# phaistos-networks/Trinity

Measured on AMD Instinct MI355X. Metric: queries/sec, higher is better.
Workload: dtype u32

## Files before the change

### trinity_amd/csrc/host/plan_host.cpp

```cpp
#include "../planner.hpp"
#include "../lucene_enc_units.hpp"
#include "lucene_encoder.hpp"
#include "perc_lower.hpp"

#include <cstdlib>
#include <memory>
#include <mutex>

namespace {
        struct HostPlan {
                BatchPlan P;
                uint8_t *block = nullptr;
                ~HostPlan() { free(block); }
        };
        void put_err(char *err, size_t cap, const std::string &s) {
                if (err && cap) {
                        const size_t n = std::min(cap - 1, s.size());
                        memcpy(err, s.data(), n);
                        err[n] = 0;
                }
        }
}

extern "C" {
void *tri_host_index_build(const uint8_t *index, uint64_t len, const uint8_t *hits, uint64_t hits_len, int codec, const uint32_t *terms3, uint64_t nterms,
                           uint32_t docs_cnt, char *err, uint64_t errcap) {
        auto H = std::make_unique<HostIndex>();
        std::string e;
        static_assert(sizeof(tri_term) == 12, "tri_term is three u32");
        if (build_host_index(index, len, hits, hits_len, codec, reinterpret_cast<const tri_term *>(terms3), nterms, docs_cnt, *H, e) != TRI_OK) {
                put_err(err, errcap, e);
                return nullptr;
        }
        return H.release();
}
void tri_host_index_free(void *h) { delete static_cast<HostIndex *>(h); }

void *tri_host_plan(void *hindex, const uint32_t *prog, uint64_t prog_len, const uint32_t *queries2, uint64_t nq, uint32_t flags, uint32_t topk, int similarity,
                    unsigned threads, const char *const *opt_names, const uint64_t *opt_values, unsigned nopt, uint32_t cus, char *err, uint64_t errcap) {
        const HostIndex &H = *static_cast<HostIndex *>(hindex);
        PlanEnv env;
        env.cus = cus ? cus : 256;
        bool use_frag_cache = false;
        for (unsigned i = 0; i < nopt; ++i) {
                const std::string n = opt_names[i];
                if (n == "frag_cache") {
                        use_frag_cache = opt_values[i] != 0;
                        continue;
                }
                tri_options &o = env.opt;
                uint64_t *slot = n == "dense_min_postings" ? &o.dense_min_postings : n == "dense_task_cost" ? &o.dense_task_cost : n == "fused" ? &o.fused
                                 : n == "fused_task_cost" ? &o.fused_task_cost : n == "fused_freq_cap" ? &o.fused_freq_cap : n == "fused_halfwords" ? &o.fused_halfwords
                                 : n == "account_needed_bytes" ? &o.account_needed_bytes : n == "planes" ? &o.planes : n == "planes_split" ? &o.planes_split
                                 : n == "plane_div" ? &o.plane_div : n == "plane_max_bytes" ? &o.plane_max_bytes : n == "probe_max_blocks" ? &o.probe_max_blocks : n == "tree_max_bytes" ? &o.tree_max_bytes : n == "tree_max_nodes" ? &o.tree_max_nodes : n == "tree_wide_min_nodes" ? &o.tree_wide_min_nodes : n == "result_bitmaps" ? &o.result_bitmaps : n == "cand_task_cost" ? &o.cand_task_cost : n == "dense_window_cost" ? &o.dense_window_cost
                                 : n == "cand_xcd" ? &o.cand_xcd : n == "planes_order" ? &o.planes_order : n == "pset_order" ? &o.pset_order : n == "scatter_bitmap_slack" ? &o.scatter_bitmap_slack : n == "phrase_task_div" ? &o.phrase_task_div : n == "plane_amortize" ? &o.plane_amortize : n == "rich_max_terms" ? &o.rich_max_terms
                                 : n == "overlap" ? &o.overlap : n == "overlap_dense_wgs" ? &o.overlap_dense_wgs : n == "overlap_cand_wgs" ? &o.overlap_cand_wgs  : nullptr;
                if (!slot) {
                        put_err(err, errcap, "unknown option " + n);
                        return nullptr;
                }
                *slot = opt_values[i];
        }
        PlanInput in;
        in.prog = prog;
        in.prog_len = prog_len;
        static_assert(sizeof(tri_query) == 8, "tri_query is two u32");
        in.queries = reinterpret_cast<const tri_query *>(queries2);
        in.nq = nq;
        in.flags = flags;
        in.topk = topk;
        in.similarity = similarity;
        auto hp = std::make_unique<HostPlan>();
        std::unique_ptr<HostPool> pool;
        if (threads > 1)
                pool = std::make_unique<HostPool>(threads);
        std::string e;
        static trip::FragCache g_frag_cache;
        static std::mutex g_frag_mu;
        std::unique_lock<std::mutex> frag_lock(g_frag_mu, std::defer_lock);
        if (use_frag_cache)
                frag_lock.lock();
        const int rc = plan_batch(
                H, env, in, pool.get(),
                [&](size_t bytes) {
                        hp->block = static_cast<uint8_t *>(aligned_alloc(64, (bytes + 63) & ~(size_t)63));
                        if (hp->block)
                                memset(hp->block, 0, bytes);
                        return hp->block;
                },
                hp->P, e, use_frag_cache ? &g_frag_cache : nullptr);
        if (rc != TRI_OK) {
                put_err(err, errcap, e);
                return nullptr;
        }
        return hp.release();
}
void tri_host_plan_free(void *p) { delete static_cast<HostPlan *>(p); }

void tri_host_plan_summary(void *p, uint64_t *out , double *ms ) {
        const BatchPlan &P = static_cast<HostPlan *>(p)->P;
        const uint64_t v[] = {P.block_bytes,       P.plan.size(),    P.qterms.size(),      P.tasks.size(),  P.fused.size(),       P.qplane.size(),    P.plane_terms.size(), P.sterms.size(),
                              P.sweights.size(),   P.phrases.size(), P.pterms.size(),      P.ptasks.size(), P.plan.off,           P.qterms.off,       P.tasks.off,          P.sched.off,
                              P.fused.off,         P.qplane.off,     P.plane_terms.off,    P.sterms.off,    P.sweights.off,       P.phrases.off,      P.pterms.off,         P.ptasks.off,
                              P.n_dense,           P.n_cand,         P.n_fused,            P.n_fused16,     P.n_fusedgen,         P.n_planes,         P.n_planes8,          P.plw,
                              P.sparse_cap,        P.out_capacity,   P.term_bytes,         P.term_bytes_dense, P.dense_queries,   P.cand_queries,     P.fused_queries,      P.planes_queries,
                              P.unsupported_queries, P.rich_R,       sizeof(DevQuery),     sizeof(DevTask), sizeof(DevFused),     sizeof(DevPhrase),  P.cand_needed_term_bytes, P.plane_decoded_bytes,
                              P.n_pset,            P.pset_queries,   P.n_probe,            P.probe_queries, P.units.size(),       P.units.off,        P.pset_sched.off,     sizeof(DevPsetUnit),
                              P.n_tree,            P.tree_queries,   P.tree.size(),        P.tree.off,      P.tree_terms.size(),  P.tree_terms.off,   P.tree_hidden.size(), P.tree_hidden.off,
// ... 190 lines not shown
```

### trinity_amd/csrc/planner.hpp

```cpp
#pragma once
#include "planner_lower.hpp"
#include "planner_tasks.hpp"

namespace trip {
        struct RowQ {
                uint8_t n = 0, q[CAND_QUEUES] = {}, sub[CAND_QUEUES] = {};
        };
        struct LapTimer {
                const bool on;
                std::chrono::steady_clock::time_point t0 = std::chrono::steady_clock::now();
                std::string line;
                void lap(const char *what) {
                        if (!on)
                                return;
                        char buf[64];
                        snprintf(buf, sizeof buf, " %s %.3f", what, ms_since(t0));
                        line += buf;
                }
        };

        struct PlanState {
                const HostIndex &ix;
                const PlanEnv &env;
                const tri_options &opt;
// ... 235 lines not shown
                        q.out_off += f.b_off;
                        if (f.tmp[i].fuse)
                                q.fused_idx += (uint32_t)f.b_fused;
                        if (f.tmp[i].tree)
                                q.fused_idx += (uint32_t)f.b_tree;
                        if (f.tmp[i].hidden) {
                                q.qid = 0xffffffffu;
                                P.tree_hidden[f.b_hidden + f.tmp[i].hidden_ord] = (uint32_t)(f.b_plan + i);
                        } else
                                P.slot_of_query[q.qid] = (uint32_t)(f.b_plan + i);
                        P.plan[f.b_plan + i] = q;
                }
                if (!f.treepool.empty()) {
                        memcpy(&P.tree[f.b_tree], f.treepool.data(), f.treepool.size() * 4);
                        for (size_t i = 0; i < f.tmp.size(); ++i) {
                                if (!f.tmp[i].tree)
                                        continue;
                                uint32_t *rec = &P.tree[f.b_tree + f.tmp[i].q.fused_idx];
                                DevTreeNode *tn = reinterpret_cast<DevTreeNode *>(rec + TREE_HDR_WORDS);
                                for (uint32_t k = 0; k < rec[0]; ++k)
                                        if (tn[k].op == TRI_OP_TERM)
                                                tn[k].row = (uint32_t)(std::lower_bound(P.tree_terms.begin(), P.tree_terms.end(), tn[k].arg) - P.tree_terms.begin());
                                        else if (tn[k].op == TRI_OP_PHRASE) {
                                                tn[k].arg += (uint32_t)f.b_plan;
                                                tn[k].row += (uint32_t)f.b_hidden;
                                        }
                        }
                }
                for (size_t i = 0; i < f.tasks.size(); ++i) {
                        DevTask t = f.tasks[i];
                        t.slot += (uint32_t)f.b_plan;
                        t.out_off += f.b_off;
                        P.tasks[f.b_tasks + i] = t;
                }
                if (!f.qterms.empty())
                        memcpy(&P.qterms[f.b_qterms], f.qterms.data(), f.qterms.size() * 4);
                if (!f.sterms.empty())
                        memcpy(&P.sterms[f.b_sterms], f.sterms.data(), f.sterms.size() * 4);
                if (S.C.scored && !f.sweights.empty())
                        memcpy(&P.sweights[f.b_sterms], f.sweights.data(), f.sweights.size() * 8);
                for (size_t i = 0; i < f.phrases.size(); ++i) {
                        DevPhrase ph = f.phrases[i];
                        ph.term_base += (uint32_t)f.b_pterms;
                        P.phrases[f.b_phrases + i] = ph;
                }
                if (!f.pterms.empty())
                        memcpy(&P.pterms[f.b_pterms], f.pterms.data(), f.pterms.size() * 4);
                for (size_t i = 0; i < f.ptasks.size(); ++i)
                        P.ptasks[f.b_ptasks + i] = f.ptasks[i] + (uint32_t)f.b_tasks;
                for (size_t i = 0; i < f.fused.size(); ++i)
                        P.fused[f.b_fused + i] = f.fused[i];
                for (const FUse &u : f.fuses)
                        P.fused[f.b_fused + u.fidx].plane[u.slot] = row_of_rank[ix.df_rank[u.term]];
                for (size_t i = 0; i < f.units.size(); ++i) {
                        DevPsetUnit u = f.units[i];
                        u.out_off += f.b_off;
                        u.tix += (uint32_t)f.b_tasks;
                        u.term_base += (uint32_t)f.b_qterms;
                        const bool is_probe = f.tasks[f.units[i].tix].kind == TASK_PROBE;
                        bool rows = true;
                        for (uint32_t k = is_probe ? 1u : 0u; k < u.nterms; ++k) {
                                const uint32_t term = (k < PSET_INLINE_TERMS ? u.tt[k] : f.qterms[f.units[i].term_base + k]) & QT_TERM;
                                const uint32_t rank = ix.df_rank[term];
                                const uint32_t row = rank < row_of_rank.size() ? row_of_rank[rank] : PL_NONE;
                                rows &= row != PL_NONE;
                                if (k < PSET_INLINE_TERMS)
                                        u.row[k] = row;
                                if (row == PL_NONE && (u.first & PSET_UNIT_SCATTER) && u.w_begin == 0)
                                        f.pscatter_docs += ix.terms[term].documents;
                        }
                        if (is_probe && !rows) {
                                P.tasks[u.tix].kind = TASK_CAND;
                                if (u.first & PSET_UNIT_FIRST) {
                                        ++f.probe_demoted;
                                        f.probe_demoted_bytes += distinct_docbytes(ix, &f.qterms[f.units[i].term_base], u.nterms, f.S.seen);
                                }
                        }
                        P.units[f.b_units + i] = u;
                        S.unit_of_task[u.tix] = (uint32_t)(f.b_units + i);
                }
                if (S.n.splane) {
                        std::fill(&P.splane.p[f.b_sterms], &P.splane.p[f.b_sterms] + f.sterms.size(), PL_NONE);
                        for (const QUse &u : f.suses)
                                P.splane[f.b_sterms + u.qpos] = row_of_rank[ix.df_rank[u.term]];
                }
                if (S.n.qplane) {
                        std::fill(&P.qplane.p[f.b_qterms], &P.qplane.p[f.b_qterms] + f.qterms.size(), PL_NONE);
                        for (const QUse &u : f.quses)
                                P.qplane[f.b_qterms + u.qpos] = row_of_rank[ix.df_rank[u.term]];
                }
                return TRI_OK;
        }

        inline uint32_t key_planes_order(const PlanState &S, const Frag &f, const size_t i, const DevTask &tk) {
                const DevQuery &q = S.P.plan[tk.slot];
                const DevFused &z = S.P.fused[q.fused_idx];
                uint32_t minrow = PL_NONE;
                for (uint32_t sidx = 0; sidx < z.nslots; ++sidx)
                        minrow = std::min(minrow, z.plane[sidx]);
                const uint32_t ord = (uint32_t)(f.b_tasks + i) - q.first_task, per = SCHED_NB / 4;
                return SCHED_RANK[tk.kind] * SCHED_NB + (S.opt.planes_order == 2 ? std::min(minrow, per - 1) * 4 + std::min(ord, 3u) : std::min(ord, 3u) * per + std::min(minrow, per - 1));
        }
        inline uint32_t key_pset_order(const PlanState &S, const Frag &f, const size_t i) {
                const uint32_t range = (uint32_t)(f.tcost[i] & 0xffffffffull) / PSET_TASK_WINDOWS;
                const uint32_t rb = S.pset_ranges <= PSET_RANGE_BKS ? std::min(range, PSET_RANGE_BKS - 1) : (uint32_t)std::min<uint64_t>((uint64_t)range * PSET_RANGE_BKS / S.pset_ranges, PSET_RANGE_BKS - 1);
                return PSET_KEY0 + rb * PSET_SUBS + pset_sub((uint32_t)(f.tcost[i] >> 32));
        }
        inline uint32_t key_cand_rows(const PlanState &S, const Frag &f, const size_t i, const DevTask &tk) {
                const DevQuery &q = S.P.plan[tk.slot];
                uint32_t row = PL_NONE;
                for (uint32_t k = 1; k < q.nterms && row == PL_NONE; ++k)
                        row = S.P.qplane[q.term_base + k];
                uint32_t queue, sub;
                if (tk.tile_end - tk.tile_begin > CAND_HEAVY_TILES || row == PL_NONE)
                        queue = (uint32_t)(f.b_tasks + i) % CAND_QUEUES, sub = (sched_key(TASK_CAND, f.tcost[i]) % SCHED_NB) / (SCHED_NB / CAND_COST_SUBS);
                else if (row < S.rowq.size() && S.rowq[row].n) {
                        const RowQ &z = S.rowq[row];
                        const uint32_t piece = (uint32_t)(f.b_tasks + i) % z.n;
                        queue = z.q[piece], sub = z.sub[piece];
                } else
                        queue = row % CAND_QUEUES, sub = CAND_SUBS - 1;
                return CAND_KEY0 + queue * CAND_SUBS + sub;
        }
// ... 240 lines not shown
```

### trinity_amd/csrc/planner_lower.hpp

```cpp
#pragma once
#include "planner_types.hpp"

namespace trip {
        inline int parse_program(const HostIndex &ix, const uint32_t *prog, uint32_t len, Scratch &S) {
                auto &nodes = S.nodes;
                auto &st = S.st;
                auto &pool = S.kidpool;
                nodes.clear();
                st.clear();
                pool.clear();
                for (uint32_t i = 0; i < len; ++i) {
                        const uint32_t op = prog[i] >> 28, arg = prog[i] & 0x0fffffffu;
                        PNode n;
                        n.op = op;
                        n.tok = i;
                        if (op == TRI_OP_TERM) {
                                n.term = arg;
                                n.cost = arg < ix.terms.size() ? ix.terms[arg].documents : 0;
                                n.empty = n.cost == 0;
                        } else {
                                const uint32_t nk = op == TRI_OP_SOME ? (arg & 0xffffu) : arg;
                                if (nk < 1 || nk > st.size())
                                        return -1;
                                S.tmpk.assign(st.end() - nk, st.end());
// ... 519 lines not shown
                                        ++g;
                        }
                        const uint32_t sidx = slot_of(tt & QT_TERM);
                        if (in_not)
                                z.nmask |= fm << (sidx * z.fbits);
                        else {
                                z.gmask[g] |= fm << (sidx * z.fbits);
                                z.gslots[g] |= 1u << sidx;
                        }
                }
                z.nreq = (uint32_t)(g + 1);
                if (z.nreq >= 1 && nreq_groups <= FUS_MAX_SLOTS) {
                        t.fz = (int32_t)f.fz.size();
                        f.fz.push_back(z);
                }
        }

        inline void classify(const Ctx &C, Frag &f, Tmp &t, const uint64_t lead_docs) {
                const HostIndex &ix = C.ix;
                const tri_options &opt = C.env.opt;
                const auto &uniq = f.S.uniq;
                t.sumdf = 0;
                t.lead_docs = lead_docs;
                t.last_doc = 0xffffffffu;
                t.dense = uniq.size() >= 2;
                uint32_t glast = 0;
                bool in_neg = false;
                for (size_t k = 0; k < uniq.size(); ++k) {
                        const DevTerm &tk = ix.terms[uniq[k] & QT_TERM];
                        t.sumdf += tk.documents;
                        t.dense &= tk.nblocks <= lead_docs;
                        if (k && (uniq[k] & QT_GROUP)) {
                                t.last_doc = std::min(t.last_doc, glast);
                                glast = 0;
                                in_neg = uniq[k] & QT_NOT;
                        }
                        if (!in_neg)
                                glast = std::max(glast, ix.blk_last[tk.first_block + tk.nblocks - 1]);
                }
                if (!in_neg)
                        t.last_doc = std::min(t.last_doc, glast);
                t.dense &= t.sumdf >= opt.dense_min_postings;
                t.dense |= t.nlead > 1;
                const bool fusable = t.fz >= 0;
                t.fuse = t.truth || (t.dense && fusable && (opt.fused != 2 || f.fz[t.fz].nreq == 1));
                if (t.fuse) {
                        ++f.onepass_queries;
                        const DevFused &z = f.fz[t.fz];
                        for (uint32_t sidx = 0; sidx < z.nslots; ++sidx)
                                f.fused_postings += ix.terms[z.term[sidx]].documents;
                }
        }

        inline int lower_query(const Ctx &C, Frag &f, const size_t qi, const uint32_t *prog, const uint32_t plen, const double *wq, const bool hidden) {
                const HostIndex &ix = C.ix;
                const bool rich = C.rich && !hidden;
                Scratch &S = f.S;
                const int root = parse_program(ix, prog, plen, S);
                if (root < 0)
                        return herr(f.err, TRI_ERR_INVALID, "query %zu: malformed postfix program", qi);
                if (S.nodes[root].empty)
                        return TRI_OK;
                TruthPlan tp;
                bool truth = false;
                if (!extract_cnf(C, f, root, wq)) {
                        if (!build_truth(S, root, tp))
                                return hidden ? herr(f.err, TRI_ERR_INVALID, "query %zu: a phrase leaf that is not a phrase", qi) : lower_tree(C, f, qi, prog, plen, wq, root);
                        truth = true;
                        S.gt = tp.slots;
                        S.gs.assign({0u, (uint32_t)S.gt.size()});
                        S.negs.clear();
                        S.leaves = tp.leaves;
                        S.leaf_tok = tp.leaf_tok;
                        S.qphrases.clear();
                        S.phterms.clear();
                }
                order_groups(ix, S);
                const auto &uniq = S.uniq;
                if (uniq.size() > MAX_QTERMS)
                        return hidden ? herr(f.err, TRI_ERR_INVALID, "query %zu: a phrase of more than %u terms", qi, MAX_QTERMS) : lower_tree(C, f, qi, prog, plen, wq, root);
                S.rt.clear();
                if (rich) {
                        reportable_terms(S, prog, plen);
                        if (S.rt.size() > RICH_NARROW_TERMS) {
                                if (S.rt.size() <= C.env.opt.rich_max_terms)
                                        return lower_tree(C, f, qi, prog, plen, wq, root);
                                f.left_out.push_back(qi);
                                herr(f.err, TRI_ERR_UNSUPPORTED, "query %zu: more than %u reportable terms", qi, (unsigned)C.env.opt.rich_max_terms);
                                return TRI_OK;
                        }
                }
                const uint32_t g0 = S.gorder[0];
                const uint32_t nlead = S.gs[g0 + 1] - S.gs[g0];
                const uint64_t lead_docs = group_docs(ix, S, g0);
                Tmp t{};
                if (!S.qphrases.empty() && ix.codec == TRI_CODEC_LUCENE && !ix.has_hdir)
                        return herr(f.err, TRI_ERR_INVALID, "query %zu: phrase over a LUCENE segment that was uploaded without hits.data", qi);
                emit_phrases_and_scorers(C, f, t, wq, rich);
                t.fz = -1;
                t.truth = truth;
                if (truth)
                        slot_map_from_truth(C, f, t, tp, rich);
                else if (C.scored && C.in.topk && S.qphrases.empty() && C.env.opt.fused)
                        slot_map_from_cnf(C, f, t);
                t.q.fused_idx = 0;
                t.q.form = RESULT_DOCIDS;
                t.q.nterms = (uint32_t)uniq.size();
                t.q.term_base = (uint32_t)f.qterms.size();
                t.q.out_cap = 0;
                t.q.out_off = 0;
                t.q.qid = (uint32_t)qi;
                t.nlead = nlead;
                f.qterms.insert(f.qterms.end(), uniq.begin(), uniq.end());
                f.term_bytes += distinct_docbytes(ix, uniq.data(), uniq.size(), S.seen);
                t.cost = 0;
                for (size_t i = 0; i < uniq.size(); ++i) {
                        const DevTerm &tk = ix.terms[uniq[i] & QT_TERM];
                        t.cost += i < nlead ? tk.documents : 32ull * std::min<uint64_t>(tk.nblocks, lead_docs);
                }
                classify(C, f, t, lead_docs);
                t.hidden = hidden;
                f.tmp.push_back(t);
                return TRI_OK;
        }

        inline int lower_range(const Ctx &C, Frag &f) {
                const PlanInput &in = C.in;
                const HostIndex &ix = C.ix;
                constexpr size_t AHEAD = 6;
                auto prefetch_query = [&](const size_t q) { for_each_term_token(ix, in, q, [&](const uint32_t x) { prefetch_term(ix, x); }); };
                auto prefetch_tails = [&](const size_t q) {
                        for_each_term_token(ix, in, q, [&](const uint32_t x) {
                                const DevTerm &tk = ix.terms[x];
                                if (tk.nblocks)
                                        __builtin_prefetch(&ix.blk_last[tk.first_block + tk.nblocks - 1]);
                        });
                };
                for (size_t q = f.q_lo; q < std::min(f.q_hi, f.q_lo + AHEAD); ++q)
                        prefetch_query(q);
                for (size_t qi = f.q_lo; qi < f.q_hi; ++qi) {
                        if (qi + AHEAD < f.q_hi)
                                prefetch_query(qi + AHEAD);
                        if (qi + AHEAD / 2 < f.q_hi)
                                prefetch_tails(qi + AHEAD / 2);
                        const tri_query &tq = in.queries[qi];
                        if ((uint64_t)tq.prog_off + tq.prog_len > in.prog_len || !tq.prog_len)
                                return herr(f.err, TRI_ERR_INVALID, "query %zu: program slice out of range", qi);
                        if (const int rc = lower_query(C, f, qi, in.prog + tq.prog_off, tq.prog_len, in.weights ? in.weights + tq.prog_off : nullptr, false))
                                return rc;
                }
                return TRI_OK;
        }

        inline int lower_tree(const Ctx &C, Frag &f, const size_t qi, const uint32_t *prog, const uint32_t plen, const double *wq, const int root) {
                const HostIndex &ix = C.ix;
// ... 288 lines not shown
```

### trinity_amd/csrc/planner_tasks.hpp

```cpp
#pragma once
#include "planner_types.hpp"

namespace trip {
        inline void tasks_tree(const Ctx &C, Frag &f, Tmp &t, const uint32_t slot, uint64_t &off) {
                t.q.out_off = off;
                t.q.out_cap = (uint32_t)t.tree_ub;
                t.q.first_task = (uint32_t)f.tasks.size();
                t.q.ntasks = 1;
                f.tcost.push_back(std::max<uint64_t>(1, t.tree_ub));
                f.tasks.push_back({slot, 0, (C.plw + TREE_CHUNK_WORDS - 1) / TREE_CHUNK_WORDS, TASK_TREE, off});
                off += t.q.out_cap;
                ++f.tree_queries;
        }

        inline int tasks_onepass(const Ctx &C, Frag &f, Tmp &t, const uint32_t slot, uint64_t &off) {
                const HostIndex &ix = C.ix;
                DevFused z = f.fz[t.fz];
                uint32_t nsparse = 0;
                for (uint32_t sidx = 0; sidx < z.nslots; ++sidx) {
                        z.plane[sidx] = PL_NONE;
                        nsparse += C.plane_ok(z.term[sidx]) ? 0u : 1u;
                }
                const bool pk = !t.truth && (C.env.opt.planes & 4u) && nsparse <= PLK_MAX_SPARSE && ix.max_doc < 0x7fff0000u;
                {
// ... 130 lines not shown
                if (C.scored && (planes_opt & 1u))
                        for (uint32_t k = 0; k < t.q.nscore; ++k) {
                                const uint32_t term = f.sterms[t.q.score_base + k];
                                if (C.plane_ok(term)) {
                                        f.benefit[ix.df_rank[term]] += std::min<uint64_t>(ix.terms[term].documents, 32ull * t.lead_docs);
                                        f.suses.push_back({t.q.score_base + k, term});
                                }
                        }
                return r;
        }

        inline int tasks_windows(const Ctx &C, Frag &f, Tmp &t, const uint32_t slot, const uint32_t *qt, const Route r, const uint64_t off) {
                const HostIndex &ix = C.ix;
                const tri_options &opt = C.env.opt;
                const uint32_t nlead = t.nlead;
                const bool pset = r.pset, pscatter = r.pscatter;
                const uint32_t nwin = t.last_doc / SPAN_BITS + 1;
                bool bitmap = false;
                double est = 1.0;
                if (pset || (C.mode == TRI_FLAG_DOCUMENTS_ONLY && opt.result_bitmaps && !t.q.nphrases)) {
                        const double N = std::max<double>(1.0, (double)ix.info.docs_cnt);
                        double g = 0.0;
                        bool negg = false;
                        for (uint32_t k = 0; k <= t.q.nterms; ++k) {
                                if (k == t.q.nterms || (k && (qt[k] & QT_GROUP))) {
                                        if (!negg)
                                                est *= std::min(1.0, g / N);
                                        g = 0.0;
                                }
                                if (k == t.q.nterms)
                                        break;
                                if (qt[k] & QT_GROUP)
                                        negg = qt[k] & QT_NOT;
                                g += ix.terms[qt[k] & QT_TERM].documents;
                        }
                        bitmap = C.mode == TRI_FLAG_DOCUMENTS_ONLY && opt.result_bitmaps && !t.q.nphrases && (pscatter || est * N >= (double)nwin * SPAN_WORDS);
                }
                uint32_t round_win = 1;
                while (round_win < PSET_TASK_WINDOWS && est * (double)PSET_ROUND_DOCS * (double)(round_win * 2u) <= 0.75 * (double)PSET_STAGE_DOCS)
                        round_win *= 2u;
                if (pscatter && !bitmap)
                        return herr(f.err, TRI_ERR_INTERNAL, "query %u: a scatter union whose result is not a bitmap", t.q.qid);
                t.q.form = bitmap ? RESULT_BITMAP : RESULT_DOCIDS;
                const uint64_t per_win = std::max<uint64_t>(1, t.sumdf / (ix.info.docs_cnt / SPAN_BITS + 1)) + (pset ? 0 : opt.dense_window_cost);
                const uint32_t pdiv = t.q.nphrases ? (uint32_t)std::max<uint64_t>(1, C.phrase_task_div) : 1u;
                const uint32_t win_per_task = pset ? std::max(1u, PSET_TASK_WINDOWS / pdiv) : (uint32_t)std::max<uint64_t>(1, std::max<uint64_t>(1, opt.dense_task_cost) / pdiv / per_win);
                uint32_t ord = 0;
                uint64_t lead_blocks = 0;
                for (uint32_t k = 0; k < nlead; ++k)
                        lead_blocks += ix.terms[qt[k] & QT_TERM].nblocks;
                uint64_t heaviest = 0xffffffffull;
                for (uint32_t k = 0; pset && k < t.q.nterms; ++k)
                        heaviest = std::min<uint64_t>(heaviest, ix.df_rank[qt[k] & QT_TERM]);
                for (uint32_t wb = 0; wb < nwin; wb += win_per_task, ++ord) {
                        const uint32_t we = std::min(nwin, wb + win_per_task);
                        uint64_t b1 = 0;
                        for (uint32_t k = 0; k < nlead; ++k)
                                b1 += C.first_block_ge(ix.terms[qt[k] & QT_TERM], (uint64_t)wb * SPAN_BITS);
                        f.tcost.push_back(pset ? wb | heaviest << 32 : per_win * (we - wb));
                        const uint64_t task_off = bitmap ? off + (uint64_t)wb * SPAN_WORDS : off + b1 * 32 + 32ull * ord * nlead;
                        if (pset)
                                f.units.push_back(make_unit(t.q, qt, (uint32_t)f.tasks.size(), wb, we, task_off,
                                                            (bitmap ? PSET_UNIT_BITMAP : 0u) | (pscatter ? PSET_UNIT_SCATTER : 0u) | round_win << PSET_UNIT_ROUND_SHIFT));
                        f.tasks.push_back({slot, wb, we, pset ? TASK_PSET : TASK_DENSE, task_off});
                }
                t.q.out_cap = bitmap ? nwin * SPAN_WORDS : (uint32_t)std::min<uint64_t>(0xffffffffull, lead_blocks * 32 + 32ull * (ord + 1) * nlead);
                f.bitmap_queries += bitmap;
                f.pscatter_queries += pscatter;
                return TRI_OK;
        }

        inline uint64_t cand_needed_bytes(const HostIndex &ix, const uint32_t *qt, const uint32_t nterms) {
                const DevTerm &lead = ix.terms[qt[0] & QT_TERM];
                uint64_t need = ix.docbytes[qt[0] & QT_TERM];
                const uint32_t *ll = &ix.blk_last[lead.first_block];
                for (uint32_t k = 1; k < nterms; ++k) {
                        const DevTerm &tk = ix.terms[qt[k] & QT_TERM];
                        const uint32_t *ol = &ix.blk_last[tk.first_block];
                        uint64_t blocks = 0;
                        uint32_t at = 0;
                        for (uint32_t lb = 0; lb < lead.nblocks && at < tk.nblocks; ++lb) {
                                const uint32_t lo_doc = lb ? ll[lb - 1] + 1 : 1u, hi_doc = ll[lb];
                                at = (uint32_t)(std::lower_bound(ol + at, ol + tk.nblocks, lo_doc) - ol);
                                if (at >= tk.nblocks)
                                        break;
                                const uint32_t last = (uint32_t)(std::lower_bound(ol + at, ol + tk.nblocks, hi_doc) - ol);
                                const uint32_t span = std::min(last, tk.nblocks - 1) - at + 1;
                                const uint32_t ndocs = lb + 1 == lead.nblocks ? lead.last_n : 32u;
                                blocks += std::min(span, ndocs);
                        }
                        need += (uint64_t)((double)ix.docbytes[qt[k] & QT_TERM] * std::min(1.0, (double)blocks / std::max(1u, tk.nblocks)));
                }
                return need;
        }

        inline void tasks_tiles(const Ctx &C, Frag &f, Tmp &t, const uint32_t slot, const uint32_t *qt, const Route r, const uint64_t off) {
                const tri_options &opt = C.env.opt;
                const DevTerm &lead = C.ix.terms[qt[0] & QT_TERM];
                const uint32_t ntiles = (lead.nblocks + TILE_BLOCKS - 1) / TILE_BLOCKS;
                const uint64_t per_tile = std::max<uint64_t>(1, t.cost / ntiles);
                const uint32_t tiles_per_task = (uint32_t)std::max<uint64_t>(1, std::max<uint64_t>(1, opt.cand_task_cost / (t.q.nphrases ? std::max<uint64_t>(1, C.phrase_task_div) : 1)) / per_tile);
                for (uint32_t tb = 0; tb < ntiles; tb += tiles_per_task) {
                        const uint32_t te = std::min(ntiles, tb + tiles_per_task);
                        f.tcost.push_back(per_tile * (te - tb));
                        if (r.probe)
                                f.units.push_back(make_unit(t.q, qt, (uint32_t)f.tasks.size(), tb, te, off + (uint64_t)tb * TILE_CANDS, tb == 0 ? PSET_UNIT_FIRST : 0u));
                        f.tasks.push_back({slot, tb, te, r.probe ? TASK_PROBE : TASK_CAND, off + (uint64_t)tb * TILE_CANDS});
                }
                t.q.out_cap = lead.documents;
                if (opt.account_needed_bytes)
                        f.cand_needed_term_bytes += cand_needed_bytes(C.ix, qt, t.q.nterms);
        }

        inline int task_range(const Ctx &C, Frag &f) {
                const HostIndex &ix = C.ix;
                f.benefit.assign(C.n_ok, 0);
                f.cand_row.assign(C.n_ok, 0);
                uint64_t off = 0;
                for (size_t ti = 0; ti < f.tmp.size(); ++ti) {
                        if (ti + 6 < f.tmp.size()) {
                                const Tmp &a = f.tmp[ti + 6];
                                for (uint32_t k = 0; k < a.q.nterms && k < 8 && !a.tree; ++k)
                                        prefetch_term(ix, f.qterms[a.q.term_base + k] & QT_TERM);
                        }
                        Tmp &t = f.tmp[ti];
                        const uint32_t slot = (uint32_t)ti;
                        if (t.tree) {
                                tasks_tree(C, f, t, slot, off);
                                continue;
                        }
                        if (t.fuse) {
                                if (const int rc = tasks_onepass(C, f, t, slot, off))
                                        return rc;
                                continue;
                        }
                        const uint32_t *qt = &f.qterms[t.q.term_base];
                        const Route r = route_cnf(C, f, t, qt);
                        t.q.out_off = off;
                        t.q.first_task = (uint32_t)f.tasks.size();
                        if (t.dense) {
                                if (const int rc = tasks_windows(C, f, t, slot, qt, r, off))
                                        return rc;
                        } else
                                tasks_tiles(C, f, t, slot, qt, r, off);
                        off += t.q.out_cap;
                        t.q.ntasks = (uint32_t)f.tasks.size() - t.q.first_task;
                        if (t.q.nphrases)
                                for (uint32_t k = t.q.first_task; k < t.q.first_task + t.q.ntasks; ++k)
                                        f.ptasks.push_back(k);
                }
                f.off = off;
                return TRI_OK;
        }
}
```

### trinity_amd/csrc/planner_types.hpp

```cpp
#pragma once
#include "host_pool.hpp"
#include "index_host.hpp"

#include <array>
#include <chrono>
#include <cmath>
#include <memory>
#include <numeric>

struct tri_options {
        uint64_t dense_min_postings = 512 * 1024;
        uint64_t dense_task_cost = 192 * 1024;
        uint64_t dense_window_cost = 16 * 1024;
        uint64_t cand_task_cost = 32 * 1024;
        uint64_t fused = 1;
        uint64_t fused_task_cost = 0;
        uint64_t fused_freq_cap = 0;
        uint64_t account_needed_bytes = 0;
        uint64_t fused_halfwords = 1;
        uint64_t overlap_dense_wgs = 0, overlap_cand_wgs = 0;
        uint64_t overlap = 0;
        uint64_t planes = 7;
        uint64_t planes_split = 0;
        uint64_t plane_div = 1024;
        uint64_t plane_amortize = 1;
        uint64_t plane_max_bytes = 8ull << 30;
        uint64_t planes_rebuild = 0;
        uint64_t phrase_task_div = 0;
        uint64_t planes_order = 1;
        uint64_t scatter_bitmap_slack = 4;
        uint64_t pset_order = 1;
        uint64_t cand_xcd = 1;
        uint64_t plan_threads = 0;
        uint64_t plan_hot_us = 300;
        uint64_t plan_pin = 2;
        uint64_t result_bitmaps = 1;
        uint64_t tree_max_bytes = 16ull << 30;
        uint64_t tree_max_nodes = 64;
        uint64_t tree_wide_min_nodes = 65;
        uint64_t rich_max_terms = 16;
        uint64_t isect_max_bytes = 2ull << 30;
        uint64_t isect_max_masks = 262144;
        uint64_t isect_max_runs = 524288;
        uint64_t perc_max_bytes = 4ull << 30;
        uint64_t perc_prune = 1;
        uint64_t probe_max_blocks = 0;
};

struct PlanEnv {
        tri_options opt;
        uint32_t cus = 256;
        uint32_t fus_wgs_per_cu = 2;
        uint32_t plk_wgs_per_cu = 2;
};

template <class T>
struct Span {
        T *p = nullptr;
        size_t n = 0;
        size_t off = 0;
        size_t size() const { return n; }
        bool empty() const { return !n; }
        T *data() { return p; }
        const T *data() const { return p; }
        T &operator[](size_t i) { return p[i]; }
        const T &operator[](size_t i) const { return p[i]; }
        T *begin() { return p; }
        T *end() { return p + n; }
        const T *begin() const { return p; }
        const T *end() const { return p + n; }
};

struct PlanInput {
        const uint32_t *prog = nullptr;
        size_t prog_len = 0;
        const tri_query *queries = nullptr;
        size_t nq = 0;
        const double *weights = nullptr;
        uint32_t flags = 0, topk = 0;
        int similarity = TRI_SIM_BM25;
};

namespace trip {
        struct PlanCounters {
                uint64_t term_bytes = 0, term_bytes_dense = 0, term_bytes_fused = 0, term_bytes_planes = 0, term_bytes_phrase_hits = 0, term_bytes_pset = 0, term_bytes_probe = 0,
                         cand_needed_term_bytes = 0;
                uint64_t dense_queries = 0, pset_queries = 0, probe_queries = 0, cand_queries = 0, fused_queries = 0, planes_queries = 0, tree_queries = 0;
                uint64_t bitmap_queries = 0;
                uint64_t pscatter_queries = 0, pscatter_docs = 0;
                uint64_t cand_lead_docs = 0, cand_terms = 0;
                uint64_t probe_demoted = 0, probe_demoted_bytes = 0;
                uint32_t sparse_cap = 0;
                uint32_t rich_R = 0;
                uint64_t rich_wide_queries = 0;
                bool rich_allow = false;
                void merge(const PlanCounters &o) {
                        term_bytes += o.term_bytes, term_bytes_dense += o.term_bytes_dense, term_bytes_fused += o.term_bytes_fused, term_bytes_planes += o.term_bytes_planes;
                        term_bytes_phrase_hits += o.term_bytes_phrase_hits, term_bytes_pset += o.term_bytes_pset, term_bytes_probe += o.term_bytes_probe;
// ... 196 lines not shown
                uint64_t off = 0;
                size_t b_plan = 0, b_qterms = 0, b_sterms = 0, b_phrases = 0, b_pterms = 0, b_tasks = 0, b_fused = 0, b_ptasks = 0, b_units = 0, b_tree = 0, b_hidden = 0;
                uint64_t b_off = 0;
                int rc = TRI_OK;
                std::string err;
                void recycle() {
                        Frag fresh;
                        auto keep = [](auto &dst, auto &src) {
                                src.clear();
                                dst = std::move(src);
                        };
                        keep(fresh.S.nodes, S.nodes), keep(fresh.S.kidpool, S.kidpool), keep(fresh.S.st, S.st), keep(fresh.S.tmpk, S.tmpk), keep(fresh.S.cs, S.cs);
                        keep(fresh.S.gt, S.gt), keep(fresh.S.gs, S.gs), keep(fresh.S.gorder, S.gorder), keep(fresh.S.leaves, S.leaves), keep(fresh.S.leaf_tok, S.leaf_tok);
                        keep(fresh.S.negs, S.negs), keep(fresh.S.opts, S.opts), keep(fresh.S.opt_tok, S.opt_tok), keep(fresh.S.ts, S.ts), keep(fresh.S.ts_tok, S.ts_tok);
                        keep(fresh.S.u, S.u), keep(fresh.S.uniq, S.uniq), keep(fresh.S.rt, S.rt), keep(fresh.S.seen, S.seen), keep(fresh.S.phterms, S.phterms);
                        keep(fresh.S.slots, S.slots), keep(fresh.S.qphrases, S.qphrases), keep(fresh.S.sc, S.sc);
                        keep(fresh.tmp, tmp), keep(fresh.qterms, qterms), keep(fresh.pterms, pterms), keep(fresh.sterms, sterms), keep(fresh.sweights, sweights);
                        keep(fresh.phrases, phrases), keep(fresh.fz, fz), keep(fresh.left_out, left_out), keep(fresh.tasks, tasks), keep(fresh.tcost, tcost);
                        keep(fresh.fused, fused), keep(fresh.ptasks, ptasks), keep(fresh.units, units), keep(fresh.quses, quses), keep(fresh.suses, suses);
                        keep(fresh.fuses, fuses), keep(fresh.benefit, benefit), keep(fresh.cand_row, cand_row), keep(fresh.keys, keys), keep(fresh.hist, hist), keep(fresh.treepool, treepool);
                        keep(fresh.tree_terms, tree_terms);
                        *this = std::move(fresh);
                }
        };
        struct FragCache {
                std::vector<Frag> frags;
        };

        struct Ctx {
                const HostIndex &ix;
                const PlanEnv &env;
                const PlanInput &in;
                bool scored, rich;
                uint32_t mode;
                uint32_t n_ok = 0;
                bool plane_ok(uint32_t term) const { return ix.df_rank[term] < n_ok; }
                uint64_t planes_split = 2, fused_task_cost = 0, phrase_task_div = 1;
                uint32_t plw = 0;
                double term_weight(const uint32_t df) const {
                        if (in.similarity == TRI_SIM_TFIDF)
                                return std::log((double)((uint64_t)ix.info.docs_cnt + 1) / (double)(df + 1)) + 1.0;
                        if (in.similarity == TRI_SIM_TRIVIAL)
                                return 0.0;
                        const float num = (float)((uint64_t)ix.info.docs_cnt - (uint64_t)df) + 0.5f;
                        const float den = (float)df + 0.5f;
                        return (double)std::log(1 + num / den);
                }
                uint32_t first_block_ge(const DevTerm &t, const uint64_t key) const {
                        if (t.win_off != 0xffffffffu && !ix.win.empty() && !(key & (CELL_DOCS - 1)) && (key >> CELL_LOG2) < ix.nwin)
                                return ix.win[t.win_off + (key >> CELL_LOG2)];
                        const uint32_t *lb = &ix.blk_last[t.first_block];
                        return (uint32_t)(std::lower_bound(lb, lb + t.nblocks, (uint32_t)std::min<uint64_t>(key, 0xffffffffull)) - lb);
                }
        };

        inline uint64_t distinct_docbytes(const HostIndex &ix, const uint32_t *terms, const size_t n, std::vector<uint32_t> &seen) {
                uint64_t bytes = 0;
                seen.clear();
                for (size_t k = 0; k < n; ++k) {
                        const uint32_t term = terms[k] & QT_TERM;
                        if (std::find(seen.begin(), seen.end(), term) == seen.end()) {
                                seen.push_back(term);
                                bytes += ix.docbytes[term];
                        }
                }
                return bytes;
        }
        inline DevPsetUnit make_unit(const DevQuery &q, const uint32_t *qt, const uint32_t tix, const uint32_t begin, const uint32_t end, const uint64_t out_off, const uint32_t first) {
                DevPsetUnit u{};
                u.out_off = out_off;
                u.first = first;
                u.w_begin = begin, u.w_end = end;
                u.tix = tix;
                u.nterms = q.nterms;
                u.term_base = q.term_base;
                for (uint32_t k = 0; k < q.nterms && k < PSET_INLINE_TERMS; ++k)
                        u.tt[k] = qt[k];
                return u;
        }
        template <class Fn>
        inline void for_each_term_token(const HostIndex &ix, const PlanInput &in, const size_t q, Fn &&fn) {
                const tri_query &t = in.queries[q];
                if ((uint64_t)t.prog_off + t.prog_len > in.prog_len)
                        return;
                for (uint32_t i = 0; i < t.prog_len && i < 16; ++i) {
                        const uint32_t tok = in.prog[t.prog_off + i];
                        const uint32_t x = tok & 0x0fffffffu;
                        if ((tok >> 28) == TRI_OP_TERM && x < ix.terms.size())
                                fn(x);
                }
        }
        inline void prefetch_term(const HostIndex &ix, const uint32_t x) {
                __builtin_prefetch(&ix.terms[x]);
                __builtin_prefetch(&ix.docbytes[x]);
                __builtin_prefetch(&ix.df_rank[x]);
        }

        inline double ms_since(std::chrono::steady_clock::time_point &t0) {
                const auto now = std::chrono::steady_clock::now();
                const double ms = std::chrono::duration<double, std::milli>(now - t0).count();
                t0 = now;
                return ms;
        }
}
```

### trinity_amd/csrc/trinity_hip.hip

```cpp
#include "../../include/trinity_hip.h"
#include <chrono>
#include <hip/hip_runtime.h>

#include <algorithm>
#include <array>
#include <cmath>
#include <cstdarg>
#include <cstdio>
#include <cstring>
#include <ctime>
#include <unistd.h>
#include <dlfcn.h>
#include <memory>
#include <mutex>
#include <numeric>
#include <string>
#include <thread>
#include <unordered_map>
#include <functional>
#include <vector>

static thread_local char g_err[512] = "";
static int fail(int code, const char *fmt, ...) {
        va_list ap;
// ... 412 lines not shown
        HIP_TRY(hipGetDeviceCount(&n));
        if (device < 0 || device >= n)
                return fail(TRI_ERR_INVALID, "tri_dev_open: device %d out of range (%d devices)", device, n);
        HIP_TRY(hipSetDevice(device));
        auto d = std::make_unique<tri_dev>();
        d->device = device;
        HIP_TRY(hipStreamCreateWithFlags(&d->stream, hipStreamNonBlocking));
        HIP_TRY(hipStreamCreateWithFlags(&d->stream2, hipStreamNonBlocking));
        HIP_TRY(hipStreamCreateWithFlags(&d->stream_up, hipStreamNonBlocking));
        HIP_TRY(hipStreamCreateWithFlags(&d->stream_rb, hipStreamNonBlocking));
        HIP_TRY(hipEventCreateWithFlags(&d->ev_fork, hipEventDisableTiming));
        HIP_TRY(hipEventCreateWithFlags(&d->ev_join, hipEventDisableTiming));
        hipDeviceProp_t prop;
        HIP_TRY(hipGetDeviceProperties(&prop, device));
        d->cus = prop.multiProcessorCount;
        *out = d.release();
        return TRI_OK;
}

extern "C" void tri_dev_close(tri_dev *d) {
        if (!d)
                return;
        if (d->refs > 0) {
                d->closing = true;
                return;
        }
        dev_destroy(d);
}

namespace {
        uint64_t *option_slot(tri_options &o, const char *name) {
                static const struct {
                        const char *name;
                        uint64_t tri_options::*field;
                } table[] = {{"dense_min_postings", &tri_options::dense_min_postings}, {"dense_task_cost", &tri_options::dense_task_cost},
                             {"fused", &tri_options::fused},
                             {"fused_task_cost", &tri_options::fused_task_cost},
                             {"fused_freq_cap", &tri_options::fused_freq_cap},
                             {"fused_halfwords", &tri_options::fused_halfwords},
                             {"account_needed_bytes", &tri_options::account_needed_bytes},
                             {"overlap_dense_wgs", &tri_options::overlap_dense_wgs},
                             {"overlap_cand_wgs", &tri_options::overlap_cand_wgs},
                             {"overlap", &tri_options::overlap},
                             {"planes", &tri_options::planes},
                             {"plane_div", &tri_options::plane_div},
                             {"planes_split", &tri_options::planes_split},
                             {"plane_max_bytes", &tri_options::plane_max_bytes},
                             {"plane_amortize", &tri_options::plane_amortize},
                             {"planes_rebuild", &tri_options::planes_rebuild},
                             {"cand_xcd", &tri_options::cand_xcd},
                             {"plan_threads", &tri_options::plan_threads},
                             {"probe_max_blocks", &tri_options::probe_max_blocks}, {"phrase_task_div", &tri_options::phrase_task_div}, {"plan_hot_us", &tri_options::plan_hot_us}, {"plan_pin", &tri_options::plan_pin}, {"planes_order", &tri_options::planes_order}, {"pset_order", &tri_options::pset_order}, {"scatter_bitmap_slack", &tri_options::scatter_bitmap_slack}, {"tree_max_bytes", &tri_options::tree_max_bytes}, {"tree_max_nodes", &tri_options::tree_max_nodes}, {"tree_wide_min_nodes", &tri_options::tree_wide_min_nodes}, {"rich_max_terms", &tri_options::rich_max_terms}, {"result_bitmaps", &tri_options::result_bitmaps}, {"cand_task_cost", &tri_options::cand_task_cost}, {"dense_window_cost", &tri_options::dense_window_cost},
                             {"isect_max_bytes", &tri_options::isect_max_bytes}, {"isect_max_masks", &tri_options::isect_max_masks}, {"isect_max_runs", &tri_options::isect_max_runs},
                             {"perc_max_bytes", &tri_options::perc_max_bytes}, {"perc_prune", &tri_options::perc_prune}};
                for (const auto &e : table)
                        if (!strcmp(e.name, name))
                                return &(o.*(e.field));
                return nullptr;
        }
}

extern "C" int tri_dev_set_option(tri_dev *d, const char *name, uint64_t value) {
        if (!d || !name)
                return fail(TRI_ERR_INVALID, "tri_dev_set_option: null argument");
        uint64_t *slot = option_slot(d->opt, name);
        if (!slot)
                return fail(TRI_ERR_INVALID, "tri_dev_set_option: unknown option '%s'", name);
        *slot = value;
        return TRI_OK;
}

extern "C" int tri_dev_get_option(tri_dev *d, const char *name, uint64_t *value) {
        if (!d || !name || !value)
                return fail(TRI_ERR_INVALID, "tri_dev_get_option: null argument");
        if (!strcmp(name, "rich_write_last_us") || !strcmp(name, "rank_last_us")) {
                *value = !strcmp(name, "rich_write_last_us") ? d->rich_write_last_us : d->rank_last_us;
                return TRI_OK;
        }
        for (int i = 0; i < CONSUMER_COUNT; ++i)
                if (!strcmp(name, CONSUMER_LAST_US[i])) {
                        *value = d->consumer_last_us[i];
                        return TRI_OK;
                }
        if (!strcmp(name, "crank_merge_last_us")) {
                *value = d->crank_merge_last_us;
                return TRI_OK;
        }
        const uint64_t *slot = option_slot(d->opt, name);
        if (!slot)
                return fail(TRI_ERR_INVALID, "tri_dev_get_option: unknown option '%s'", name);
        *value = *slot;
        return TRI_OK;
}

extern "C" int tri_dev_memory(tri_dev *d, tri_dev_memory_info *out) {
        if (!d || !out)
                return fail(TRI_ERR_INVALID, "tri_dev_memory: null argument");
        HIP_TRY(hipSetDevice(d->device));
        size_t fr = 0, total = 0;
        HIP_TRY(hipMemGetInfo(&fr, &total));
        DevLock g(d->mu);
        uint64_t all = 0, pinned = 0;
        for (const auto &kv : d->pool.size_of)
                all += kv.second;
        for (const auto &pb : d->pinned_idle)
                pinned += pb.first;
        out->pool_idle_bytes = d->pool.idle_bytes;
// ... 2045 lines not shown
```

Baseline: 14.72 million.

## Speed up host planner: flat-query fast path, batched task emission, row reuse

Adds a plan_fast option, on by default, that lowers flat AND/OR term-only queries directly without the general parse and grouping path. Task and unit emission now sizes the vectors once and fills them in place instead of pushing one element at a time. Block-window entries are prefetched before the binary searches. Row lookup is skipped for consecutive pset units that share the same terms. These cut CPU-side planning cost, which counts toward queries/sec, at the risk of the fast path diverging from the general lowering, for example in term ordering or group flags.

```diff
diff --git a/trinity_amd/csrc/host/plan_host.cpp b/trinity_amd/csrc/host/plan_host.cpp
--- a/trinity_amd/csrc/host/plan_host.cpp
+++ b/trinity_amd/csrc/host/plan_host.cpp
@@ -53,7 +53,7 @@
                                  : n == "fused_task_cost" ? &o.fused_task_cost : n == "fused_freq_cap" ? &o.fused_freq_cap : n == "fused_halfwords" ? &o.fused_halfwords
                                  : n == "account_needed_bytes" ? &o.account_needed_bytes : n == "planes" ? &o.planes : n == "planes_split" ? &o.planes_split
                                  : n == "plane_div" ? &o.plane_div : n == "plane_max_bytes" ? &o.plane_max_bytes : n == "probe_max_blocks" ? &o.probe_max_blocks : n == "tree_max_bytes" ? &o.tree_max_bytes : n == "tree_max_nodes" ? &o.tree_max_nodes : n == "tree_wide_min_nodes" ? &o.tree_wide_min_nodes : n == "result_bitmaps" ? &o.result_bitmaps : n == "cand_task_cost" ? &o.cand_task_cost : n == "dense_window_cost" ? &o.dense_window_cost
-                                 : n == "cand_xcd" ? &o.cand_xcd : n == "planes_order" ? &o.planes_order : n == "pset_order" ? &o.pset_order : n == "scatter_bitmap_slack" ? &o.scatter_bitmap_slack : n == "phrase_task_div" ? &o.phrase_task_div : n == "plane_amortize" ? &o.plane_amortize : n == "rich_max_terms" ? &o.rich_max_terms
+                                 : n == "cand_xcd" ? &o.cand_xcd : n == "planes_order" ? &o.planes_order : n == "pset_order" ? &o.pset_order : n == "scatter_bitmap_slack" ? &o.scatter_bitmap_slack : n == "phrase_task_div" ? &o.phrase_task_div : n == "plane_amortize" ? &o.plane_amortize : n == "rich_max_terms" ? &o.rich_max_terms : n == "plan_fast" ? &o.plan_fast
                                  : n == "overlap" ? &o.overlap : n == "overlap_dense_wgs" ? &o.overlap_dense_wgs : n == "overlap_cand_wgs" ? &o.overlap_cand_wgs  : nullptr;
                 if (!slot) {
                         put_err(err, errcap, "unknown option " + n);
diff --git a/trinity_amd/csrc/planner.hpp b/trinity_amd/csrc/planner.hpp
--- a/trinity_amd/csrc/planner.hpp
+++ b/trinity_amd/csrc/planner.hpp
@@ -311,14 +311,18 @@
                         P.fused[f.b_fused + i] = f.fused[i];
                 for (const FUse &u : f.fuses)
                         P.fused[f.b_fused + u.fidx].plane[u.slot] = row_of_rank[ix.df_rank[u.term]];
+                bool prev_rows = true;
                 for (size_t i = 0; i < f.units.size(); ++i) {
                         DevPsetUnit u = f.units[i];
                         u.out_off += f.b_off;
                         u.tix += (uint32_t)f.b_tasks;
                         u.term_base += (uint32_t)f.b_qterms;
                         const bool is_probe = f.tasks[f.units[i].tix].kind == TASK_PROBE;
-                        bool rows = true;
-                        for (uint32_t k = is_probe ? 1u : 0u; k < u.nterms; ++k) {
+                        const bool again = i && u.w_begin && f.units[i - 1].term_base == f.units[i].term_base && f.units[i - 1].nterms == u.nterms;
+                        if (again)
+                                memcpy(u.row, P.units[f.b_units + i - 1].row, sizeof u.row);
+                        bool rows = again ? prev_rows : true;
+                        for (uint32_t k = is_probe ? 1u : 0u; k < u.nterms && !again; ++k) {
                                 const uint32_t term = (k < PSET_INLINE_TERMS ? u.tt[k] : f.qterms[f.units[i].term_base + k]) & QT_TERM;
                                 const uint32_t rank = ix.df_rank[term];
                                 const uint32_t row = rank < row_of_rank.size() ? row_of_rank[rank] : PL_NONE;
@@ -328,6 +332,7 @@
                                 if (row == PL_NONE && (u.first & PSET_UNIT_SCATTER) && u.w_begin == 0)
                                         f.pscatter_docs += ix.terms[term].documents;
                         }
+                        prev_rows = rows;
                         if (is_probe && !rows) {
                                 P.tasks[u.tix].kind = TASK_CAND;
                                 if (u.first & PSET_UNIT_FIRST) {
diff --git a/trinity_amd/csrc/planner_lower.hpp b/trinity_amd/csrc/planner_lower.hpp
--- a/trinity_amd/csrc/planner_lower.hpp
+++ b/trinity_amd/csrc/planner_lower.hpp
@@ -595,10 +595,76 @@
                 }
         }
 
+        inline int record_query(const Ctx &C, Frag &f, size_t qi, const double *wq, bool rich, bool hidden, const TruthPlan *tp, uint32_t nlead, uint64_t lead_docs);
+
+        inline bool lower_flat(const Ctx &C, Frag &f, const size_t qi, const uint32_t *prog, const uint32_t plen, const double *wq, const bool rich, int &rc) {
+                if (plen < 3 || plen > MAX_QTERMS + 1)
+                        return false;
+                const uint32_t n = plen - 1, op = prog[n] >> 28;
+                if ((op != TRI_OP_AND && op != TRI_OP_OR) || (prog[n] & 0x0fffffffu) != n)
+                        return false;
+                const HostIndex &ix = C.ix;
+                const size_t known = ix.terms.size();
+                uint32_t term[MAX_QTERMS], docs[MAX_QTERMS], ord[MAX_QTERMS];
+                for (uint32_t i = 0; i < n; ++i) {
+                        const uint32_t x = prog[i] & 0x0fffffffu;
+                        if ((prog[i] >> 28) != TRI_OP_TERM || x >= known)
+                                return false;
+                        for (uint32_t j = 0; j < i; ++j)
+                                if (term[j] == x)
+                                        return false;
+                        term[i] = x;
+                        docs[i] = ix.terms[x].documents;
+                }
+                rc = TRI_OK;
+                uint32_t live = 0, nlead = 1;
+                uint64_t lead_docs = 0;
+                if (op == TRI_OP_AND) {
+                        for (uint32_t a = 0; a < n; ++a) {
+                                if (!docs[a])
+                                        return true;
+                                uint32_t b = a;
+                                for (; b && docs[ord[b - 1]] > docs[a]; --b)
+                                        ord[b] = ord[b - 1];
+                                ord[b] = a;
+                        }
+                        live = n;
+                        lead_docs = docs[ord[0]];
+                } else {
+                        for (uint32_t i = 0; i < n; ++i)
+                                if (docs[i]) {
+                                        ord[live++] = i;
+                                        lead_docs += docs[i];
+                                }
+                        if (!live)
+                                return true;
+                        nlead = live;
+                }
+                Scratch &S = f.S;
+                S.uniq.clear(), S.leaves.clear(), S.leaf_tok.clear(), S.rt.clear(), S.qphrases.clear(), S.phterms.clear();
+                for (uint32_t k = 0; k < live; ++k) {
+                        S.uniq.push_back(term[ord[k]] | (op == TRI_OP_AND || k == 0 ? QT_GROUP : 0u));
+                        if (C.scored) {
+                                S.leaves.push_back(term[ord[k]]);
+                                S.leaf_tok.push_back(ord[k]);
+                        }
+                }
+                for (uint32_t i = 0; rich && i < n; ++i)
+                        if (docs[i])
+                                S.rt.push_back(term[i]);
+                rc = record_query(C, f, qi, wq, rich, false, nullptr, nlead, lead_docs);
+                return true;
+        }
+
         inline int lower_query(const Ctx &C, Frag &f, const size_t qi, const uint32_t *prog, const uint32_t plen, const double *wq, const bool hidden) {
                 const HostIndex &ix = C.ix;
                 const bool rich = C.rich && !hidden;
                 Scratch &S = f.S;
+                if (C.env.opt.plan_fast && !hidden) {
+                        int rc = TRI_OK;
+                        if (lower_flat(C, f, qi, prog, plen, wq, rich, rc))
+                                return rc;
+                }
                 const int root = parse_program(ix, prog, plen, S);
                 if (root < 0)
                         return herr(f.err, TRI_ERR_INVALID, "query %zu: malformed postfix program", qi);
@@ -634,8 +700,15 @@
                         }
                 }
                 const uint32_t g0 = S.gorder[0];
-                const uint32_t nlead = S.gs[g0 + 1] - S.gs[g0];
-                const uint64_t lead_docs = group_docs(ix, S, g0);
+                return record_query(C, f, qi, wq, rich, hidden, truth ? &tp : nullptr, S.gs[g0 + 1] - S.gs[g0], group_docs(ix, S, g0));
+        }
+
+        inline int record_query(const Ctx &C, Frag &f, const size_t qi, const double *wq, const bool rich, const bool hidden, const TruthPlan *tp, const uint32_t nlead,
+                                const uint64_t lead_docs) {
+                const HostIndex &ix = C.ix;
+                Scratch &S = f.S;
+                const auto &uniq = S.uniq;
+                const bool truth = tp != nullptr;
                 Tmp t{};
                 if (!S.qphrases.empty() && ix.codec == TRI_CODEC_LUCENE && !ix.has_hdir)
                         return herr(f.err, TRI_ERR_INVALID, "query %zu: phrase over a LUCENE segment that was uploaded without hits.data", qi);
@@ -643,7 +716,7 @@
                 t.fz = -1;
                 t.truth = truth;
                 if (truth)
-                        slot_map_from_truth(C, f, t, tp, rich);
+                        slot_map_from_truth(C, f, t, *tp, rich);
                 else if (C.scored && C.in.topk && S.qphrases.empty() && C.env.opt.fused)
                         slot_map_from_cnf(C, f, t);
                 t.q.fused_idx = 0;
diff --git a/trinity_amd/csrc/planner_tasks.hpp b/trinity_amd/csrc/planner_tasks.hpp
--- a/trinity_amd/csrc/planner_tasks.hpp
+++ b/trinity_amd/csrc/planner_tasks.hpp
@@ -206,17 +206,39 @@
                 uint64_t heaviest = 0xffffffffull;
                 for (uint32_t k = 0; pset && k < t.q.nterms; ++k)
                         heaviest = std::min<uint64_t>(heaviest, ix.df_rank[qt[k] & QT_TERM]);
+                const uint32_t ntasks = (uint32_t)(((uint64_t)nwin + win_per_task - 1) / win_per_task);
+                const size_t task0 = f.tasks.size(), unit0 = f.units.size();
+                f.tasks.resize(task0 + ntasks);
+                f.tcost.resize(task0 + ntasks);
+                DevTask *const tasks = f.tasks.data() + task0;
+                uint64_t *const tcost = f.tcost.data() + task0;
+                DevPsetUnit *units = nullptr, unit{};
+                if (pset) {
+                        f.units.resize(unit0 + ntasks);
+                        units = f.units.data() + unit0;
+                        unit = make_unit(t.q, qt, 0, 0, 0, 0, (bitmap ? PSET_UNIT_BITMAP : 0u) | (pscatter ? PSET_UNIT_SCATTER : 0u) | round_win << PSET_UNIT_ROUND_SHIFT);
+                }
+                if (!bitmap)
+                        for (uint32_t wb = 0; wb < nwin; wb += win_per_task)
+                                for (uint32_t k = 0; k < nlead; ++k)
+                                        C.prefetch_block_ge(ix.terms[qt[k] & QT_TERM], (uint64_t)wb * SPAN_BITS);
                 for (uint32_t wb = 0; wb < nwin; wb += win_per_task, ++ord) {
                         const uint32_t we = std::min(nwin, wb + win_per_task);
-                        uint64_t b1 = 0;
-                        for (uint32_t k = 0; k < nlead; ++k)
-                                b1 += C.first_block_ge(ix.terms[qt[k] & QT_TERM], (uint64_t)wb * SPAN_BITS);
-                        f.tcost.push_back(pset ? wb | heaviest << 32 : per_win * (we - wb));
-                        const uint64_t task_off = bitmap ? off + (uint64_t)wb * SPAN_WORDS : off + b1 * 32 + 32ull * ord * nlead;
-                        if (pset)
-                                f.units.push_back(make_unit(t.q, qt, (uint32_t)f.tasks.size(), wb, we, task_off,
-                                                            (bitmap ? PSET_UNIT_BITMAP : 0u) | (pscatter ? PSET_UNIT_SCATTER : 0u) | round_win << PSET_UNIT_ROUND_SHIFT));
-                        f.tasks.push_back({slot, wb, we, pset ? TASK_PSET : TASK_DENSE, task_off});
+                        uint64_t task_off = off + (uint64_t)wb * SPAN_WORDS;
+                        if (!bitmap) {
+                                uint64_t b1 = 0;
+                                for (uint32_t k = 0; k < nlead; ++k)
+                                        b1 += C.first_block_ge(ix.terms[qt[k] & QT_TERM], (uint64_t)wb * SPAN_BITS);
+                                task_off = off + b1 * 32 + 32ull * ord * nlead;
+                        }
+                        tcost[ord] = pset ? wb | heaviest << 32 : per_win * (we - wb);
+                        if (pset) {
+                                unit.out_off = task_off;
+                                unit.w_begin = wb, unit.w_end = we;
+                                unit.tix = (uint32_t)(task0 + ord);
+                                units[ord] = unit;
+                        }
+                        tasks[ord] = {slot, wb, we, pset ? TASK_PSET : TASK_DENSE, task_off};
                 }
                 t.q.out_cap = bitmap ? nwin * SPAN_WORDS : (uint32_t)std::min<uint64_t>(0xffffffffull, lead_blocks * 32 + 32ull * (ord + 1) * nlead);
                 f.bitmap_queries += bitmap;
@@ -254,12 +276,19 @@
                 const uint32_t ntiles = (lead.nblocks + TILE_BLOCKS - 1) / TILE_BLOCKS;
                 const uint64_t per_tile = std::max<uint64_t>(1, t.cost / ntiles);
                 const uint32_t tiles_per_task = (uint32_t)std::max<uint64_t>(1, std::max<uint64_t>(1, opt.cand_task_cost / (t.q.nphrases ? std::max<uint64_t>(1, C.phrase_task_div) : 1)) / per_tile);
-                for (uint32_t tb = 0; tb < ntiles; tb += tiles_per_task) {
+                const uint32_t ntasks = (uint32_t)(((uint64_t)ntiles + tiles_per_task - 1) / tiles_per_task);
+                const size_t task0 = f.tasks.size();
+                f.tasks.resize(task0 + ntasks);
+                f.tcost.resize(task0 + ntasks);
+                DevTask *const tasks = f.tasks.data() + task0;
+                uint64_t *const tcost = f.tcost.data() + task0;
+                uint32_t ord = 0;
+                for (uint32_t tb = 0; tb < ntiles; tb += tiles_per_task, ++ord) {
                         const uint32_t te = std::min(ntiles, tb + tiles_per_task);
-                        f.tcost.push_back(per_tile * (te - tb));
+                        tcost[ord] = per_tile * (te - tb);
                         if (r.probe)
-                                f.units.push_back(make_unit(t.q, qt, (uint32_t)f.tasks.size(), tb, te, off + (uint64_t)tb * TILE_CANDS, tb == 0 ? PSET_UNIT_FIRST : 0u));
-                        f.tasks.push_back({slot, tb, te, r.probe ? TASK_PROBE : TASK_CAND, off + (uint64_t)tb * TILE_CANDS});
+                                f.units.push_back(make_unit(t.q, qt, (uint32_t)(task0 + ord), tb, te, off + (uint64_t)tb * TILE_CANDS, tb == 0 ? PSET_UNIT_FIRST : 0u));
+                        tasks[ord] = {slot, tb, te, r.probe ? TASK_PROBE : TASK_CAND, off + (uint64_t)tb * TILE_CANDS};
                 }
                 t.q.out_cap = lead.documents;
                 if (opt.account_needed_bytes)
diff --git a/trinity_amd/csrc/planner_types.hpp b/trinity_amd/csrc/planner_types.hpp
--- a/trinity_amd/csrc/planner_types.hpp
+++ b/trinity_amd/csrc/planner_types.hpp
@@ -44,6 +44,7 @@
         uint64_t isect_max_runs = 524288;
         uint64_t perc_max_bytes = 4ull << 30;
         uint64_t perc_prune = 1;
+        uint64_t plan_fast = 1;
         uint64_t probe_max_blocks = 0;
 };
 
@@ -346,6 +347,10 @@
                         const uint32_t *lb = &ix.blk_last[t.first_block];
                         return (uint32_t)(std::lower_bound(lb, lb + t.nblocks, (uint32_t)std::min<uint64_t>(key, 0xffffffffull)) - lb);
                 }
+                void prefetch_block_ge(const DevTerm &t, const uint64_t key) const {
+                        if (t.win_off != 0xffffffffu && !ix.win.empty() && !(key & (CELL_DOCS - 1)) && (key >> CELL_LOG2) < ix.nwin)
+                                __builtin_prefetch(&ix.win[t.win_off + (key >> CELL_LOG2)]);
+                }
         };
 
         inline uint64_t distinct_docbytes(const HostIndex &ix, const uint32_t *terms, const size_t n, std::vector<uint32_t> &seen) {
diff --git a/trinity_amd/csrc/trinity_hip.hip b/trinity_amd/csrc/trinity_hip.hip
--- a/trinity_amd/csrc/trinity_hip.hip
+++ b/trinity_amd/csrc/trinity_hip.hip
@@ -488,7 +488,7 @@
                              {"plan_threads", &tri_options::plan_threads},
                              {"probe_max_blocks", &tri_options::probe_max_blocks}, {"phrase_task_div", &tri_options::phrase_task_div}, {"plan_hot_us", &tri_options::plan_hot_us}, {"plan_pin", &tri_options::plan_pin}, {"planes_order", &tri_options::planes_order}, {"pset_order", &tri_options::pset_order}, {"scatter_bitmap_slack", &tri_options::scatter_bitmap_slack}, {"tree_max_bytes", &tri_options::tree_max_bytes}, {"tree_max_nodes", &tri_options::tree_max_nodes}, {"tree_wide_min_nodes", &tri_options::tree_wide_min_nodes}, {"rich_max_terms", &tri_options::rich_max_terms}, {"result_bitmaps", &tri_options::result_bitmaps}, {"cand_task_cost", &tri_options::cand_task_cost}, {"dense_window_cost", &tri_options::dense_window_cost},
                              {"isect_max_bytes", &tri_options::isect_max_bytes}, {"isect_max_masks", &tri_options::isect_max_masks}, {"isect_max_runs", &tri_options::isect_max_runs},
-                             {"perc_max_bytes", &tri_options::perc_max_bytes}, {"perc_prune", &tri_options::perc_prune}};
+                             {"perc_max_bytes", &tri_options::perc_max_bytes}, {"perc_prune", &tri_options::perc_prune}, {"plan_fast", &tri_options::plan_fast}};
                 for (const auto &e : table)
                         if (!strcmp(e.name, name))
                                 return &(o.*(e.field));
```

New measurement: 14.66 million. No clear change (-0.4%).
